# mmaker/c-lwe-snarks

Hardware: AMD Instinct MI355X
Metric: snark_proofs_per_sec (higher is better)
Workload: dtype u32 limbs (704-bit integers mod 2^704) + AES-256 bytes; int8 digits on the matrix cores, int32 accumulation (exact)

## Files before the change

### c-lwe-snarks_amd/csrc/evalmm.hip

```cpp
#include <algorithm>
#include <cstring>

#include "ctx.hpp"

namespace {

using mf::AesKey;

constexpr int CT = 4;
constexpr int SB = 88;
constexpr int VB = 92;
constexpr int MB = CT * SB;
constexpr int MT = MB / 32;
constexpr int RT = 128;
constexpr int TSTRIDE = 384;
constexpr int BLK_PER_ROW = 24;
static_assert(MB % 32 == 0 && CT * VB + 15 <= TSTRIDE, "tile geometry");

typedef int v4i __attribute__((ext_vector_type(4)));
typedef int v16i __attribute__((ext_vector_type(16)));

__device__ __forceinline__ uint32_t coef_at(const MmIo &io, uint32_t v, uint32_t nrows, uint32_t i) {
  if (io.bits) {
    const uint32_t a = io.bits_row0 + i;
// ... 244 lines not shown
    for (int q = 0; q < NT; q++)
#pragma unroll
      for (int e = 0; e < 16; e++) {
        const uint32_t mm = wave * 32 + (e & 3) + 8 * (e >> 2) + 4 * h;
        p[(uint64_t)mm * N + 32 * q + r32] = acc[q][e];
      }
  }
}

constexpr int RT2 = 256, TS2 = 192, BPR2 = 12, NQ2 = 16, N2 = 16 * NQ2;
template <int LOGQ> struct W16;
template <> struct W16<736> { static constexpr int CT = 2, SBY = 88, VBY = 92, MT = 11, MBP = 176, LL = 12; };
template <> struct W16<1472> { static constexpr int CT = 1, SBY = 184, VBY = 184, MT = 12, MBP = 192, LL = 23; };
static_assert(RT2 * 4 == 1024 && BPR2 % 4 == 0 && RT2 * BPR2 == 3 * 1024 && W16<736>::CT * W16<736>::VBY + 8 <= TS2 && W16<1472>::CT * W16<1472>::VBY + 8 <= TS2, "wide tile geometry");

template <int MODE, int LOGQ>
__global__ __launch_bounds__(1024) void k_evalmm16(AesKey key , const uint32_t *__restrict__ g_t0, uint64_t off,
                                                   uint32_t n, uint32_t nrows, uint32_t rows_per_chunk, const uint8_t *__restrict__ c8,
                                                   const int8_t *__restrict__ cd, int *__restrict__ part, uint8_t *__restrict__ image) {
  using G = W16<LOGQ>;
  constexpr int CT2 = G::CT, MT2 = G::MT, MB2 = G::MBP, NSW = (16 - G::MT) * 64;
  constexpr uint32_t SBq = G::SBY, VBq = G::VBY;
  struct __attribute__((aligned(16))) Lds {
    uint32_t lt[mf::kTabBytes / 4];
    uint8_t tile[RT2 * TS2];
    v4i bfrag[2][NQ2][64];
    uint32_t spanc[RT2][2][5];
  };
  __shared__ Lds lds;
  mf::lds_fill_tab(lds.lt, g_t0);
  const uint8_t *tab = reinterpret_cast<const uint8_t *>(lds.lt);
  const mf::AesLane L = mf::aes_lane();
  const uint32_t tid = threadIdx.x, lane = tid & 63, wave = tid >> 6;
  const uint32_t j0 = blockIdx.x * CT2;
  const uint32_t nks = j0 >= n ? 0u : min((uint32_t)CT2, n - j0);
  const bool has_b = j0 + CT2 > n && j0 <= n;
  const uint32_t r0 = blockIdx.y * rows_per_chunk;
  const uint32_t r1 = min(nrows, r0 + rows_per_chunk);

  v4i acc[NQ2];
#pragma unroll
  for (int q = 0; q < NQ2; q++) acc[q] = v4i{0, 0, 0, 0};

  const uint32_t c16 = lane & 15, g4 = lane >> 4;
  const uint32_t m = wave * 16 + c16;
  const uint32_t mcol = (m / SBq) * VBq + (m % SBq);
  const uint32_t hstep = (n * VBq) & 15;

  auto span_task = [&](uint32_t u0, uint32_t task) {
    const uint32_t lr = task >> 1, which = task & 1;
    const uint64_t row = (uint64_t)u0 + lr;
    if (row >= r1 || !nks) return;
    const RowGeom g = row_geom(off, row, n, j0, nks, VBq);
    const uint64_t sp0 = g.cb0 >> 8, sp1 = (g.cb0 + g.nblk - 1) >> 8;
    if (which && sp1 == sp0) return;
    uint32_t sc[5];
    mf::aes_span_consts(tab, L, key, sp0 + which, sc);
#pragma unroll
    for (int i = 0; i < 5; i++) lds.spanc[lr][which][i] = sc[i];
  };
  const v4i *cdv = reinterpret_cast<const v4i *>(cd);
  const uint32_t KS = (nrows + RT2 - 1) / RT2 * (RT2 / 64);

  __syncthreads();
  if (tid < 2 * RT2) span_task(r0, tid);
  __syncthreads();
  for (uint32_t u0 = r0; u0 < r1; u0 += RT2) {
    if (MODE == 1) {
      for (uint32_t s2 = tid; s2 < RT2 * BPR2; s2 += 1024) {
        const uint32_t lr = s2 / BPR2, k = s2 % BPR2;
        const uint64_t row = (uint64_t)u0 + lr;
        uint32_t w[4] = {0x80808080u, 0x80808080u, 0x80808080u, 0x80808080u};
        if (row < r1) {
          const RowGeom g = row_geom(off, row, n, j0, nks, VBq);
          if (k < g.nblk) {
            const uint64_t ctr = g.cb0 + k;
            const uint32_t *scp = lds.spanc[lr][(uint32_t)((ctr >> 8) - (g.cb0 >> 8))];
            uint32_t sc[5] = {scp[0], scp[1], scp[2], scp[3], scp[4]};
            mf::aes256_ctr_block_sc(tab, L, key, ctr, sc, w);
          }
        }
        *reinterpret_cast<uint4 *>(&lds.tile[lr * TS2 + 16 * k]) = make_uint4(w[0], w[1], w[2], w[3]);
      }
      __syncthreads();
      if (has_b) {
        for (uint32_t s2 = tid; s2 < RT2 * VBq; s2 += 1024) {
          const uint32_t lr = s2 / VBq, k = s2 % VBq;
          const uint64_t row = (uint64_t)u0 + lr;
          if (row >= r1) continue;
          const RowGeom g = row_geom(off, row, n, j0, nks, VBq);
          lds.tile[lr * TS2 + g.head + nks * VBq + k] = (uint8_t)(c8[row * VBq + k] ^ 0x80);
        }
        __syncthreads();
      }
      if (wave < MT2) {
        const uint32_t head0 = row_geom(off, u0, n, j0, 1, VBq).head;
        v4i *dst = reinterpret_cast<v4i *>(image) + ((uint64_t)(MT2 * blockIdx.x + wave) * KS + (u0 >> 6)) * 64 + lane;
#pragma unroll
        for (int ks = 0; ks < RT2 / 64; ks++) {
          const uint32_t lrb = ks * 64 + 16 * g4;
          uint32_t aw[4];
#pragma unroll
          for (int e4 = 0; e4 < 4; e4++) {
            uint32_t x = 0;
#pragma unroll
            for (int e = 0; e < 4; e++) {
              const uint32_t lr = lrb + 4 * e4 + e;
              x |= (uint32_t)lds.tile[lr * TS2 + ((head0 + hstep * lr) & 15) + mcol] << (8 * e);
            }
            aw[e4] = x;
          }
          dst[(uint64_t)ks * 64] = v4i{(int)aw[0], (int)aw[1], (int)aw[2], (int)aw[3]};
        }
      } else {
        const uint32_t t2 = tid - MT2 * 64;
        for (uint32_t task = t2; task < 2 * RT2; task += NSW) span_task(u0 + RT2, task);
      }
      __syncthreads();
      continue;
    }
    const v4i bstage = cdv[(uint64_t)(u0 >> 6) * NQ2 * 64 + tid];
    if (wave >= MT2) {
      const uint32_t t2 = tid - MT2 * 64;
#pragma unroll
      for (int k2 = 1; k2 < RT2 / 64; k2++)
#pragma unroll
        for (int i2 = 0; i2 < 4; i2++) {
          const uint32_t idx = t2 + NSW * i2;
          if (idx < NQ2 * 64) acc[(k2 - 1) * 4 + i2] = cdv[((uint64_t)(u0 >> 6) + k2) * NQ2 * 64 + idx];
        }
    }
    {
      const uint32_t lr = tid >> 2;
      const uint64_t row = (uint64_t)u0 + lr;
      if (row < r1) {
        const RowGeom g = row_geom(off, row, n, j0, nks, VBq);
#pragma unroll 1
        for (int it = 0; it < BPR2 / 4; it++) {
          const uint32_t k = (tid & 3) + 4 * it;
          if (k >= g.nblk) continue;
          const uint64_t ctr = g.cb0 + k;
          const uint32_t *scp = lds.spanc[lr][(uint32_t)((ctr >> 8) - (g.cb0 >> 8))];
          uint32_t sc[5] = {scp[0], scp[1], scp[2], scp[3], scp[4]};
          uint32_t w[4];
          mf::aes256_ctr_block_sc(tab, L, key, ctr, sc, w);
          *reinterpret_cast<uint4 *>(&lds.tile[lr * TS2 + 16 * k]) = make_uint4(w[0], w[1], w[2], w[3]);
        }
      }
    }
    (&lds.bfrag[0][0][0])[tid] = bstage;
    __syncthreads();
    if (has_b) {
      for (uint32_t s2 = tid; s2 < RT2 * VBq; s2 += 1024) {
        const uint32_t lr = s2 / VBq, k = s2 % VBq;
        const uint64_t row = (uint64_t)u0 + lr;
        if (row >= r1) continue;
        const RowGeom g = row_geom(off, row, n, j0, nks, VBq);
        lds.tile[lr * TS2 + g.head + nks * VBq + k] = (uint8_t)(c8[row * VBq + k] ^ 0x80);
      }
      __syncthreads();
    }
    const uint32_t head0 = row_geom(off, u0, n, j0, 1, VBq).head;
#pragma unroll
    for (int ks = 0; ks < RT2 / 64; ks++) {
      if (wave < MT2) {
        if ((uint64_t)u0 + ks * 64 < r1) {
          const uint32_t lrb = ks * 64 + 16 * g4;
          uint32_t aw[4];
#pragma unroll
          for (int e4 = 0; e4 < 4; e4++) {
            uint32_t x = 0;
#pragma unroll
            for (int e = 0; e < 4; e++) {
              const uint32_t lr = lrb + 4 * e4 + e;
              x |= (uint32_t)lds.tile[lr * TS2 + ((head0 + hstep * lr) & 15) + mcol] << (8 * e);
            }
            aw[e4] = x;
          }
          const v4i a = {(int)aw[0], (int)aw[1], (int)aw[2], (int)aw[3]};
#ifndef MM_SKIP_MFMA
#pragma unroll
          for (int q = 0; q < NQ2; q++) acc[q] = __builtin_amdgcn_mfma_i32_16x16x64_i8(a, lds.bfrag[ks & 1][q][lane], acc[q], 0, 0, 0);
#else
          acc[0][0] += a[0] + a[1] + a[2] + a[3];
#endif
        }
      } else {
        const uint32_t t2 = tid - MT2 * 64;
        if (ks + 1 < RT2 / 64) {
          v4i *dst = &lds.bfrag[(ks + 1) & 1][0][0];
#pragma unroll
          for (int i2 = 0; i2 < 4; i2++) {
            const uint32_t idx = t2 + NSW * i2;
            if (idx < NQ2 * 64) dst[idx] = acc[ks * 4 + i2];
          }
        }
        if (ks == 0)
          for (uint32_t task = t2; task < 2 * RT2; task += NSW) span_task(u0 + RT2, task);
      }
      __syncthreads();
    }
  }
  if (MODE == 0 && wave < MT2) {
    int *p = part + ((uint64_t)blockIdx.y * gridDim.x + blockIdx.x) * MB2 * N2;
#pragma unroll
    for (int q = 0; q < NQ2; q++)
#pragma unroll
      for (int e = 0; e < 4; e++) p[(uint64_t)(wave * 16 + 4 * g4 + e) * N2 + 16 * q + c16] = acc[q][e];
  }
}


#ifndef MMS_SW
#define MMS_SW 8
#endif
constexpr int SW = MMS_SW;
constexpr int TPW = 16;
#ifndef MMS_RQ
#define MMS_RQ 2
#endif
constexpr int RQ = MMS_RQ;
constexpr int RG = 16 / RQ;
constexpr int CG = SW / RG;
constexpr int CH = NQ2 / CG;
struct MmsImages { const v4i *image[16]; };
__device__ __forceinline__ void mms_item(uint32_t xcd, uint32_t slot, uint32_t ngt, uint32_t ngr, uint32_t map, uint32_t &grp, uint32_t &tg) {
  if (map == 0) {
    grp = slot % ngt;
    tg = (slot / ngt) * 8 + xcd;
  } else {
    const uint32_t blk = slot >> 5, i = slot & 31, nreg = ngt / ngr, tpb = 32 / ngr;
    grp = (blk % nreg) * ngr + i % ngr;
    tg = ((blk / nreg) * tpb + i / ngr) * 8 + xcd;
  }
}
__device__ __forceinline__ long long mms_pack_e(const v4i &a) {
  return (long long)a[0] + ((long long)a[1] << 8) + ((long long)a[2] << 16) + ((long long)a[3] << 24);
}
template <int CTRL>
__device__ __forceinline__ long long mms_quad_bcast(long long t) {
  const int lo = __builtin_amdgcn_update_dpp(0, (int)(unsigned int)(unsigned long long)t, CTRL, 0xf, 0xf, false);
  const int hi = __builtin_amdgcn_update_dpp(0, (int)((unsigned long long)t >> 32), CTRL, 0xf, 0xf, false);
  return (long long)(((unsigned long long)(unsigned int)hi << 32) | (unsigned int)lo);
}
__device__ __forceinline__ void mms_store_packed(int *__restrict__ part, uint32_t pk, uint64_t m4 , uint32_t ctile, uint32_t c16,
                                                 const v4i &acc) {
  const long long T = mms_pack_e(acc);
  if (pk == 1) {
    reinterpret_cast<long long *>(part)[m4 * N2 + 16 * ctile + c16] = T;
    return;
  }
  const long long T1 = mms_quad_bcast<0x55>(T), T2 = mms_quad_bcast<0xAA>(T), T3 = mms_quad_bcast<0xFF>(T);
  if (c16 & 3) return;
  const __int128 U = (__int128)T + (__int128)T1 * 256 + (__int128)T2 * 65536 + (__int128)T3 * 16777216;
  const unsigned __int128 u = (unsigned __int128)U;
  reinterpret_cast<uint4 *>(part)[m4 * (N2 / 4) + 4 * ctile + (c16 >> 2)] = uint4{(uint32_t)u, (uint32_t)(u >> 32), (uint32_t)(u >> 64), 0u};
}
__device__ __forceinline__ void mmstream_body(const MmsImages &imgs, uint32_t mtiles, uint32_t KS, uint32_t nrows, uint32_t rows_per_chunk,
                                              const v4i *__restrict__ cdv, int *__restrict__ part, uint32_t grp, uint32_t tg ,
                                              uint32_t chunk, uint64_t cd_stride , uint64_t part_stride , uint32_t pk ) {
  __shared__ v4i bfrag[2][RT2 / 64][NQ2][64];
  const uint32_t tid = threadIdx.x, lane = tid & 63;
  const uint32_t wave = __builtin_amdgcn_readfirstlane(tid >> 6);
  const uint32_t c16 = lane & 15, g4 = lane >> 4;
  const uint32_t rq = wave % RG, ch = wave / RG;
  if (tg * 16 >= mtiles) return;
  const v4i *__restrict__ image = imgs.image[grp];
  cdv += grp * cd_stride;
  part += grp * part_stride;
  const uint32_t mt0 = (tg * RG + rq) * RQ;
  const uint32_t r0 = chunk * rows_per_chunk, r1 = min(nrows, r0 + rows_per_chunk);
  v4i acc[RQ][CH];
#pragma unroll
  for (int t = 0; t < RQ; t++)
#pragma unroll
    for (int q = 0; q < CH; q++) acc[t][q] = v4i{0, 0, 0, 0};
  constexpr int KSN = RT2 / 64;
  constexpr int BPK = NQ2 * 64 / (SW * 64);
#ifndef MMS_DEPTH
#define MMS_DEPTH 6
#endif
  constexpr int DEPTH = MMS_DEPTH;
  auto a_load = [&](int t, uint32_t u0, int ks) -> v4i {
#ifdef MMS_SKIP_A
    return v4i{(int)u0, ks, t, (int)lane};
#endif
    const v4i *ap = image + ((uint64_t)min(mt0 + t, mtiles - 1) * KS + (u0 >> 6) + ks) * 64;
    return ap[lane];
  };
  v4i a[RQ][KSN];
  v4i bnr[KSN][BPK];
  auto b_load = [&](uint32_t u0, int ks, int i) -> v4i {
    const v4i *bp = cdv + (uint64_t)(u0 >> 6) * NQ2 * 64 + (uint64_t)ks * NQ2 * 64 + SW * 64 * i;
    return bp[tid];
  };
  if (r0 >= r1) return;
  const uint32_t ulast = r0 + (r1 - r0 - 1) / RT2 * RT2;
#pragma unroll
  for (int i = 0; i < KSN * BPK; i++) (&bfrag[0][0][0][0])[tid + SW * 64 * i] = cdv[(uint64_t)(r0 >> 6) * NQ2 * 64 + tid + SW * 64 * i];
  __builtin_amdgcn_sched_barrier(0);
#pragma unroll
  for (int ks = 0; ks < KSN; ks++) {
#pragma unroll
    for (int t = 0; t < RQ; t++) a[t][ks] = a_load(t, r0, ks);
#pragma unroll
    for (int i = 0; i < BPK; i++) bnr[ks][i] = b_load(min(r0 + RT2, ulast), ks, i);
    __builtin_amdgcn_sched_barrier(0);
  }
  __syncthreads();
#if defined(MMS_PRIO_YOUNG)
  if (wave >= SW / 2) __builtin_amdgcn_s_setprio(1);
#elif defined(MMS_PRIO_OLD)
  if (wave < SW / 2) __builtin_amdgcn_s_setprio(1);
#endif
  uint32_t buf = 0;
  for (uint32_t u0 = r0; u0 < r1; u0 += RT2) {
    const uint32_t un1 = min(u0 + RT2, ulast), un2 = min(u0 + 2 * RT2, ulast);
    const v4i *bcur = &bfrag[buf][0][ch * CH][lane];
    v4i *bnext = &bfrag[buf ^ 1][0][0][0];
    v4i ring[DEPTH];
#pragma unroll
    for (int i = 0; i < DEPTH; i++) ring[i] = bcur[((i / CH) * NQ2 + i % CH) * 64];
#pragma unroll
    for (int ks = 0; ks < KSN; ks++) {
#ifdef MMS_LOADS_ONLY
#pragma unroll
      for (int t = 0; t < RQ; t++) acc[t][ks][0] += a[t][ks][0] ^ a[t][ks][3];
#else
#pragma unroll
      for (int q = 0; q < CH; q++) {
        const int it = ks * CH + q;
        const v4i b = ring[it % DEPTH];
        if (it + DEPTH < KSN * CH) ring[it % DEPTH] = bcur[(((it + DEPTH) / CH) * NQ2 + (it + DEPTH) % CH) * 64];
#pragma unroll
        for (int t = 0; t < RQ; t++) {
#ifdef MMS_ACC_ASM
          asm volatile("v_mfma_i32_16x16x64_i8 %0, %1, %2, %0" : "+a"(acc[t][q]) : "v"(a[t][ks]), "v"(b));
#else
          acc[t][q] = __builtin_amdgcn_mfma_i32_16x16x64_i8(a[t][ks], b, acc[t][q], 0, 0, 0);
#endif
        }
        __builtin_amdgcn_sched_barrier(0);
      }
#endif
#pragma unroll
      for (int i = 0; i < BPK; i++) bnext[ks * NQ2 * 64 + tid + SW * 64 * i] = bnr[ks][i];
#pragma unroll
      for (int t = 0; t < RQ; t++) a[t][ks] = a_load(t, un1, ks);
#pragma unroll
      for (int i = 0; i < BPK; i++) bnr[ks][i] = b_load(un2, ks, i);
    }
#ifndef MMS_NOSYNC
    __syncthreads();
#endif
    buf ^= 1;
  }
  const uint64_t Mtot = (uint64_t)mtiles * 16;
#ifdef MMS_ACC_ASM
  asm volatile("s_nop 15\n\ts_nop 15" ::: "memory");
#endif
  if (pk) {
#pragma unroll
    for (int t = 0; t < RQ; t++) {
      if (mt0 + t >= mtiles) continue;
      const uint64_t m4 = (uint64_t)chunk * (Mtot / 4) + (uint64_t)(mt0 + t) * 4 + g4;
#pragma unroll
      for (int q = 0; q < CH; q++) mms_store_packed(part, pk, m4, ch * CH + q, c16, acc[t][q]);
    }
    return;
  }
#pragma unroll
  for (int t = 0; t < RQ; t++) {
    if (mt0 + t >= mtiles) continue;
    int *p = part + ((uint64_t)chunk * Mtot + (uint64_t)(mt0 + t) * 16) * N2;
#pragma unroll
    for (int q = 0; q < CH; q++)
#pragma unroll
      for (int e = 0; e < 4; e++) p[(uint64_t)(4 * g4 + e) * N2 + 16 * (ch * CH + q) + c16] = acc[t][q][e];
  }
}

__global__ __launch_bounds__(SW * 64) void k_mmstream(MmsImages imgs, uint32_t mtiles, uint32_t KS, uint32_t nrows, uint32_t rows_per_chunk,
                                                      const v4i *__restrict__ cdv, int *__restrict__ part, uint32_t ngt, uint32_t ngr, uint32_t map,
                                                      uint64_t cd_stride, uint64_t part_stride, uint32_t pk) {
  uint32_t grp, tg;
  mms_item(blockIdx.x & 7, blockIdx.x >> 3, ngt, ngr, map, grp, tg);
  mmstream_body(imgs, mtiles, KS, nrows, rows_per_chunk, cdv, part, grp, tg, blockIdx.y, cd_stride, part_stride, pk);
}
__global__ __launch_bounds__(SW * 64) void k_mmstream1(MmsImages imgs, uint32_t mtiles, uint32_t KS, uint32_t nrows, uint32_t rows_per_chunk,
                                                       const v4i *__restrict__ cdv, int *__restrict__ part, uint32_t pk) {
  mmstream_body(imgs, mtiles, KS, nrows, rows_per_chunk, cdv, part, 0u, blockIdx.x, blockIdx.y, 0, 0, pk);
}
__device__ __forceinline__ void mmstream_persistent(const MmsImages &imgs, uint32_t mtiles, uint32_t KS, uint32_t nrows, uint32_t rows_per_chunk,
                                                    const v4i *__restrict__ cdv, int *__restrict__ part, uint32_t ngt, uint32_t ngr, uint32_t map,
                                                    uint64_t cd_stride, uint64_t part_stride, uint32_t nblk , uint32_t nchunks,
                                                    uint32_t *__restrict__ sync, uint32_t sync_mode, uint32_t spin_max, uint32_t width, uint32_t pk) {
  const uint32_t xcd = blockIdx.x & 7, cu = blockIdx.x >> 3;
  const uint32_t members = sync_mode == 2 ? 32u : (map ? ngr : ngt);
  uint32_t *ctr = sync + xcd * 32 + (sync_mode == 2 ? 0u : cu / members);
  uint32_t k = 0;
  for (uint32_t chunk = 0; chunk < nchunks; chunk++)
    for (uint32_t slot = cu; slot < nblk * 32; slot += width, k++) {
      if (sync_mode && members > 1) {
        if (threadIdx.x == 0) {
          __hip_atomic_fetch_add(ctr, 1u, __ATOMIC_RELAXED, __HIP_MEMORY_SCOPE_AGENT);
          const uint32_t target = (k + 1) * members;
          for (uint32_t spin = 0; spin < spin_max && __hip_atomic_load(ctr, __ATOMIC_RELAXED, __HIP_MEMORY_SCOPE_AGENT) < target; spin++) __builtin_amdgcn_s_sleep(8);
        }
        __syncthreads();
      }
      uint32_t grp, tg;
      mms_item(xcd, slot, ngt, ngr, map, grp, tg);
      mmstream_body(imgs, mtiles, KS, nrows, rows_per_chunk, cdv, part, grp, tg, chunk, cd_stride, part_stride, pk);
    }
}
__global__ __launch_bounds__(SW * 64) void k_mmstream_p(MmsImages imgs, uint32_t mtiles, uint32_t KS, uint32_t nrows, uint32_t rows_per_chunk,
                                                        const v4i *__restrict__ cdv, int *__restrict__ part, uint32_t ngt, uint32_t ngr, uint32_t map,
                                                        uint64_t cd_stride, uint64_t part_stride, uint32_t nblk, uint32_t nchunks,
                                                        uint32_t *__restrict__ sync, uint32_t sync_mode, uint32_t spin_max, uint32_t width, uint32_t pk) {
  mmstream_persistent(imgs, mtiles, KS, nrows, rows_per_chunk, cdv, part, ngt, ngr, map, cd_stride, part_stride, nblk, nchunks, sync, sync_mode, spin_max, width, pk);
}
__global__ __launch_bounds__(SW * 64) void k_mmstream_pb(MmsImages imgs, uint32_t mtiles, uint32_t KS, uint32_t nrows, uint32_t rows_per_chunk,
                                                         const v4i *__restrict__ cdv, int *__restrict__ part, uint32_t ngt, uint32_t ngr, uint32_t map,
                                                         uint64_t cd_stride, uint64_t part_stride, uint32_t nblk, uint32_t nchunks,
                                                         uint32_t *__restrict__ sync, uint32_t sync_mode, uint32_t spin_max, uint32_t width, uint32_t pk) {
  mmstream_persistent(imgs, mtiles, KS, nrows, rows_per_chunk, cdv, part, ngt, ngr, map, cd_stride, part_stride, nblk, nchunks, sync, sync_mode, spin_max, width, pk);
}

constexpr int WSW = 4, WRQ = 4;
__device__ __forceinline__ void mfma_acc(v4i &acc, const v4i &a, const v4i &b) {
  asm volatile("v_mfma_i32_16x16x64_i8 %0, %1, %2, %0" : "+a"(acc) : "v"(a), "v"(b));
}
__device__ __forceinline__ void mmstream_body_w(const MmsImages &imgs, uint32_t mtiles, uint32_t KS, uint32_t nrows, uint32_t rows_per_chunk,
                                                const v4i *__restrict__ cdv, int *__restrict__ part, uint32_t grp, uint32_t tg, uint32_t chunk, uint64_t cd_stride,
                                                uint64_t part_stride) {
  __shared__ v4i bfrag[2][RT2 / 64][NQ2][64];
  const uint32_t tid = threadIdx.x, lane = tid & 63;
  const uint32_t wave = __builtin_amdgcn_readfirstlane(tid >> 6);
  const uint32_t c16 = lane & 15, g4 = lane >> 4;
  if (tg * 16 >= mtiles) return;
  const v4i *__restrict__ image = imgs.image[grp];
  cdv += grp * cd_stride;
  part += grp * part_stride;
  const uint32_t mt0 = tg * 16 + wave * WRQ;
  const uint32_t r0 = chunk * rows_per_chunk, r1 = min(nrows, r0 + rows_per_chunk);
  if (r0 >= r1) return;
  constexpr int KSN = RT2 / 64;
  constexpr int BPK = NQ2 * 64 / (WSW * 64);
  v4i acc[WRQ][NQ2];
#pragma unroll
  for (int t = 0; t < WRQ; t++)
#pragma unroll
    for (int q = 0; q < NQ2; q++) acc[t][q] = v4i{0, 0, 0, 0};
  auto a_load = [&](int t, uint32_t u0, int ks) -> v4i {
    const v4i *ap = image + ((uint64_t)min(mt0 + t, mtiles - 1) * KS + (u0 >> 6) + ks) * 64;
    return ap[lane];
  };
  auto b_load = [&](uint32_t u0, int ks, int i) -> v4i {
    const v4i *bp = cdv + (uint64_t)(u0 >> 6) * NQ2 * 64 + (uint64_t)ks * NQ2 * 64 + WSW * 64 * i;
    return bp[tid];
  };
  const uint32_t ulast = r0 + (r1 - r0 - 1) / RT2 * RT2;
  v4i a[WRQ][KSN], bnr[KSN][BPK];
#pragma unroll
  for (int i = 0; i < KSN * BPK; i++) (&bfrag[0][0][0][0])[tid + WSW * 64 * i] = cdv[(uint64_t)(r0 >> 6) * NQ2 * 64 + tid + WSW * 64 * i];
  __builtin_amdgcn_sched_barrier(0);
  const uint32_t ub1 = min(r0 + RT2, ulast);
#pragma unroll
  for (int i = 0; i < BPK; i++) bnr[0][i] = b_load(ub1, 0, i);
#pragma unroll
  for (int ks = 1; ks < KSN; ks++) {
#pragma unroll
    for (int i = 0; i < BPK; i++) bnr[ks][i] = b_load(ub1, ks, i);
#pragma unroll
    for (int t = 0; t < WRQ; t++) a[t][ks - 1] = a_load(t, r0, ks - 1);
    __builtin_amdgcn_sched_barrier(0);
  }
  __syncthreads();
  v4i rg[4][4];
  uint32_t buf = 0;
  auto frag = [&](uint32_t b, int f) -> v4i { return bfrag[b][f >> 4][f & 15][lane]; };
#pragma unroll
  for (int G = 0; G < 2; G++)
#pragma unroll
    for (int j = 0; j < 4; j++) rg[G][j] = frag(0, 4 * G + j);
  for (uint32_t u0 = r0; u0 < r1; u0 += RT2) {
    const uint32_t un1 = min(u0 + RT2, ulast), un2 = min(u0 + 2 * RT2, ulast);
    v4i *bnext = &bfrag[buf ^ 1][0][0][0];
#pragma unroll
    for (int ks = 0; ks < KSN; ks++) {
#pragma unroll
      for (int g = 0; g < 4; g++) {
        const int G = ks * 4 + g, Gn = G + 2;
#pragma unroll
        for (int u = 0; u < 4; u++) {
          const int j = 3 - u;
#pragma unroll
          for (int t = WRQ - 1; t >= 0; t--) mfma_acc(acc[t][4 * g + j], a[t][ks], rg[G & 3][j]);
          rg[Gn & 3][u] = Gn < 16 ? frag(buf, 4 * Gn + u) : frag(buf ^ 1, 4 * (Gn - 16) + u);
          if (g == 0) {
            bnext[ks * NQ2 * 64 + tid + WSW * 64 * (BPK - 1 - u)] = bnr[ks][BPK - 1 - u];
          } else if (g == 1) {
            bnr[ks][u] = b_load(un2, ks, u);
          } else if (g == 2) {
            if (ks == 0) a[u][KSN - 1] = a_load(u, u0, KSN - 1);
            else a[u][ks - 1] = a_load(u, un1, ks - 1);
          }
          __builtin_amdgcn_sched_barrier(0);
        }
        if (G == 9) {
          asm volatile("s_waitcnt lgkmcnt(4)\n\ts_barrier" ::: "memory");
          __builtin_amdgcn_sched_barrier(0);
        }
      }
    }
    buf ^= 1;
  }
  __syncthreads();
  asm volatile("s_nop 15\n\ts_nop 15" ::: "memory");
  const uint64_t Mtot = (uint64_t)mtiles * 16;
#pragma unroll
  for (int t = 0; t < WRQ; t++) {
    if (mt0 + t >= mtiles) continue;
    int *p = part + ((uint64_t)chunk * Mtot + (uint64_t)(mt0 + t) * 16) * N2;
#pragma unroll
    for (int q = 0; q < NQ2; q++)
#pragma unroll
      for (int e = 0; e < 4; e++) p[(uint64_t)(4 * g4 + e) * N2 + 16 * q + c16] = acc[t][q][e];
  }
}
__global__ __launch_bounds__(WSW * 64) void k_mmstream_w(MmsImages imgs, uint32_t mtiles, uint32_t KS, uint32_t nrows, uint32_t rows_per_chunk,
                                                         const v4i *__restrict__ cdv, int *__restrict__ part, uint32_t ngt, uint32_t ngr, uint32_t map,
                                                         uint64_t cd_stride, uint64_t part_stride, uint32_t nblk, uint32_t nchunks) {
  const uint32_t xcd = blockIdx.x & 7, cu = blockIdx.x >> 3;
  for (uint32_t k = 0; k < nblk * nchunks; k++) {
    uint32_t grp, tg;
    mms_item(xcd, (k % nblk) * 32 + cu, ngt, ngr, map, grp, tg);
    mmstream_body_w(imgs, mtiles, KS, nrows, rows_per_chunk, cdv, part, grp, tg, k / nblk, cd_stride, part_stride);
  }
}

template <int ND, int KWM ,
          bool PK >
__device__ __forceinline__ void evalmm_finish_body(const int *__restrict__ part, const int64_t *__restrict__ sc, uint32_t nchunks, uint32_t ntiles, uint32_t N,
                                                   uint32_t nvec, uint32_t n, uint32_t nrows, uint32_t ct, uint32_t MBv, uint32_t sby, uint32_t LL,
                                                   const MmIo &io, int accumulate, const int *__restrict__ sa_part, uint32_t sa_col) {
  __shared__ uint32_t sv[KWM][3][64];
  const uint32_t vl = threadIdx.x & 63, lq = threadIdx.x >> 6;
  const uint32_t v = blockIdx.y * 64 + vl, j = blockIdx.x;
  const uint32_t tile = j / ct, jj = j % ct;
  const uint32_t KWv = sby / 4;
  if (v < nvec) {
    int64_t corr[ND];
#pragma unroll
    for (int w = 0; w < ND; w++) corr[w] = 128 * sc[ND * v + w] + 16384ll * nrows;
    if (PK) {
      const uint64_t M4 = (uint64_t)ntiles * MBv / 4;
      unsigned __int128 corrsum = 0;
#pragma unroll
      for (int w = 0; w < ND; w++) corrsum += (unsigned __int128)((uint64_t)corr[w] * 0x01010101ull) << (8 * w);
      for (uint32_t l = lq; l < KWv; l += 4) {
        const uint64_t m4 = ((uint64_t)tile * MBv + jj * sby) / 4 + l;
        __int128 U = 0, SA = 0;
        for (uint32_t ch = 0; ch < nchunks; ch++) {
          const uint64_t at = (uint64_t)ch * M4 + m4;
          if (ND == 4) {
            const uint4 r = reinterpret_cast<const uint4 *>(part)[at * (N / 4) + v], q = reinterpret_cast<const uint4 *>(sa_part)[at * (N / 4) + sa_col / 4];
            U += (__int128)(((unsigned __int128)(uint64_t)(int64_t)(int32_t)r.z << 64) | ((uint64_t)r.y << 32) | r.x);
            SA += (__int128)(((unsigned __int128)(uint64_t)(int64_t)(int32_t)q.z << 64) | ((uint64_t)q.y << 32) | q.x);
          } else {
            U += reinterpret_cast<const long long *>(part)[at * N + v];
            SA += reinterpret_cast<const long long *>(sa_part)[at * N + sa_col];
          }
        }
        const unsigned __int128 val = (unsigned __int128)(U + SA * (__int128)(ND == 4 ? 128ll * 0x01010101ll : 128ll)) + corrsum;
        sv[l][0][vl] = (uint32_t)val;
        sv[l][1][vl] = (uint32_t)(val >> 32);
        sv[l][2][vl] = (uint32_t)(val >> 64);
      }
    } else
    for (uint32_t l = lq; l < KWv; l += 4) {
      unsigned __int128 val = 0;
      int g0[4][ND], sa0[4];
#pragma unroll
      for (int k = 0; k < 4; k++) {
        const int *row = part + ((uint64_t)tile * MBv + (jj * sby + 4 * l + k)) * N;
#pragma unroll
        for (int w = 0; w < ND; w++) g0[k][w] = row[ND * v + w];
        sa0[k] = (sa_part + ((uint64_t)tile * MBv + (jj * sby + 4 * l + k)) * N)[sa_col];
      }
#pragma unroll
      for (int k = 0; k < 4; k++) {
        const uint32_t mm = jj * sby + 4 * l + k;
        int64_t g[ND], sa = sa0[k];
#pragma unroll
        for (int w = 0; w < ND; w++) g[w] = g0[k][w];
        for (uint32_t ch = 1; ch < nchunks; ch++) {
          const int *row = part + (((uint64_t)ch * ntiles + tile) * MBv + mm) * N;
#pragma unroll
          for (int w = 0; w < ND; w++) g[w] += row[ND * v + w];
          sa += (sa_part + (((uint64_t)ch * ntiles + tile) * MBv + mm) * N)[sa_col];
        }
        uint64_t t = 0;
#pragma unroll
        for (int w = 0; w < ND; w++) t += (uint64_t)(g[w] + 128 * sa + corr[w]) << (8 * w);
        val += (unsigned __int128)t << (8 * k);
      }
      sv[l][0][vl] = (uint32_t)val;
      sv[l][1][vl] = (uint32_t)(val >> 32);
      sv[l][2][vl] = (uint32_t)(val >> 64);
    }
  }
  __syncthreads();
  if (lq != 0 || v >= nvec) return;
  uint32_t *out = reinterpret_cast<uint32_t *>((v < io.osplit ? io.out[0] + (uint64_t)v * io.ostride : io.out[1] + (uint64_t)(v - io.osplit) * io.ostride) +
                                               (uint64_t)j * LL);
  const bool wide4 = (LL & 1) == 0 && (io.ostride & 1) == 0 && ((reinterpret_cast<uintptr_t>(io.out[0]) | reinterpret_cast<uintptr_t>(io.out[1])) & 15) == 0;
  uint32_t pend[4] = {0, 0, 0, 0};
  uint64_t carry = 0;
  const uint32_t *actw = io.add_ct ? reinterpret_cast<const uint32_t *>(io.add_ct + (uint64_t)j * LL) : nullptr;
  const uint64_t ax = io.add_ct ? io.add_scale[v] : 0;
  uint64_t acarry = 0;
  for (uint32_t l = 0; l < KWv; l++) {
    uint64_t word = carry + sv[l][0][vl];
    if (l >= 1) word += sv[l - 1][1][vl];
    if (l >= 2) word += sv[l - 2][2][vl];
    if (accumulate) word += out[l];
    if (actw) {
      const uint64_t t = (uint64_t)actw[l] * ax + acarry;
      word += (uint32_t)t;
      acarry = t >> 32;
    }
    carry = word >> 32;
    pend[l & 3] = (uint32_t)word;
    if (wide4 ? (l & 3) == 3 : (l & 1) == 1) {
      if (wide4) *reinterpret_cast<uint4 *>(out + (l & ~3u)) = uint4{pend[0], pend[1], pend[2], pend[3]};
      else *reinterpret_cast<uint2 *>(out + (l & ~1u)) = uint2{pend[(l & 2)], pend[(l & 2) + 1]};
    }
  }
  if (wide4) {
    if (KWv & 3) *reinterpret_cast<uint4 *>(out + (KWv & ~3u)) = uint4{pend[0], (KWv & 3) > 1 ? pend[1] : 0u, (KWv & 3) > 2 ? pend[2] : 0u, 0u};
    for (uint32_t l = (KWv + 3) & ~3u; l < 2 * LL; l += 4) *reinterpret_cast<uint4 *>(out + l) = uint4{0u, 0u, 0u, 0u};
  } else {
    if (KWv & 1) *reinterpret_cast<uint2 *>(out + (KWv & ~1u)) = uint2{pend[(KWv & 2)], 0u};
    for (uint32_t l = (KWv + 1) & ~1u; l < 2 * LL; l += 2) *reinterpret_cast<uint2 *>(out + l) = uint2{0u, 0u};
  }
}

template <int ND, int KWM, bool PK>
__global__ __launch_bounds__(256) void k_evalmm_finish(const int *__restrict__ part, const int64_t *__restrict__ sc, uint32_t nchunks, uint32_t ntiles,
                                                        uint32_t N, uint32_t nvec, uint32_t n, uint32_t nrows, uint32_t ct, uint32_t MBv, uint32_t sby,
                                                        uint32_t LL, MmIo io, int accumulate) {
  evalmm_finish_body<ND, KWM, PK>(part, sc, nchunks, ntiles, N, nvec, n, nrows, ct, MBv, sby, LL, io, accumulate, part, ND * nvec);
}
template <int ND, int KWM, bool PK>
__global__ __launch_bounds__(256) void k_evalmm_finish_groups(const int *__restrict__ part, uint64_t part_stride, uint32_t nchunks, uint32_t ntiles, uint32_t N,
                                                               uint32_t n, uint32_t nrows, uint32_t ct, uint32_t MBv, uint32_t sby, uint32_t LL, MmGroupArgs A,
                                                               int accumulate) {
  const uint32_t g = blockIdx.z, lender = A.io[g].sa_from1 ? A.io[g].sa_from1 - 1 : g;
// ... 385 lines not shown
```

Baseline: 14000.

## Carry LDS ring prefetch across tiles and replace block sync with mid-step barrier

Hoists the B-fragment LDS ring out of the tile loop so the prefetch of the next tile's fragments overlaps the tail of the current tile. The LDS stores and global B loads are spread across the q iterations of the MFMA loop instead of being bunched after it. The end-of-tile __syncthreads is replaced by an explicit s_waitcnt lgkmcnt plus s_barrier placed at a computed slot. This is meant to hide LDS and global latency and shorten barrier stalls, but the hand-placed barrier and counter depend on static geometry assumptions and risk races if those assumptions are wrong.

```diff
diff --git a/c-lwe-snarks_amd/csrc/evalmm.hip b/c-lwe-snarks_amd/csrc/evalmm.hip
--- a/c-lwe-snarks_amd/csrc/evalmm.hip
+++ b/c-lwe-snarks_amd/csrc/evalmm.hip
@@ -570,9 +570,9 @@
 #pragma unroll
   for (int ks = 0; ks < KSN; ks++) {
 #pragma unroll
+    for (int i = 0; i < BPK; i++) bnr[ks][i] = b_load(min(r0 + RT2, ulast), ks, i);
+#pragma unroll
     for (int t = 0; t < RQ; t++) a[t][ks] = a_load(t, r0, ks);
-#pragma unroll
-    for (int i = 0; i < BPK; i++) bnr[ks][i] = b_load(min(r0 + RT2, ulast), ks, i);
     __builtin_amdgcn_sched_barrier(0);
   }
   __syncthreads();
@@ -581,25 +581,35 @@
 #elif defined(MMS_PRIO_OLD)
   if (wave < SW / 2) __builtin_amdgcn_s_setprio(1);
 #endif
+  [[maybe_unused]] constexpr int NF = KSN * CH;
+  [[maybe_unused]] constexpr int BSLOT = 2 * CH + CH - 1 - DEPTH;
+  static_assert(DEPTH >= 1 && DEPTH + BPK <= CH && 2 * BPK <= CH, "the stage barrier follows the ds_writes of its k-step and that k-step's last ring read");
+  static_assert(CH - DEPTH - BPK <= 15, "lgkmcnt is a 4-bit count");
+  v4i ring[DEPTH];
+#pragma unroll
+  for (int i = 0; i < DEPTH; i++) {
+    ring[i] = bfrag[0][i / CH][ch * CH + i % CH][lane];
+    __builtin_amdgcn_sched_barrier(0);
+  }
   uint32_t buf = 0;
   for (uint32_t u0 = r0; u0 < r1; u0 += RT2) {
     const uint32_t un1 = min(u0 + RT2, ulast), un2 = min(u0 + 2 * RT2, ulast);
-    const v4i *bcur = &bfrag[buf][0][ch * CH][lane];
+    [[maybe_unused]] const v4i *bcur = &bfrag[buf][0][ch * CH][lane];
+    [[maybe_unused]] const v4i *bnxt = &bfrag[buf ^ 1][0][ch * CH][lane];
     v4i *bnext = &bfrag[buf ^ 1][0][0][0];
-    v4i ring[DEPTH];
-#pragma unroll
-    for (int i = 0; i < DEPTH; i++) ring[i] = bcur[((i / CH) * NQ2 + i % CH) * 64];
 #pragma unroll
     for (int ks = 0; ks < KSN; ks++) {
+#pragma unroll
+      for (int q = 0; q < CH; q++) {
 #ifdef MMS_LOADS_ONLY
-#pragma unroll
-      for (int t = 0; t < RQ; t++) acc[t][ks][0] += a[t][ks][0] ^ a[t][ks][3];
+        if (q == 0) {
+#pragma unroll
+          for (int t = 0; t < RQ; t++) acc[t][ks][0] += a[t][ks][0] ^ a[t][ks][3];
+        }
 #else
-#pragma unroll
-      for (int q = 0; q < CH; q++) {
-        const int it = ks * CH + q;
+        const int it = ks * CH + q, nx = it + DEPTH;
         const v4i b = ring[it % DEPTH];
-        if (it + DEPTH < KSN * CH) ring[it % DEPTH] = bcur[(((it + DEPTH) / CH) * NQ2 + (it + DEPTH) % CH) * 64];
+        ring[it % DEPTH] = nx < NF ? bcur[((nx / CH) * NQ2 + nx % CH) * 64] : bnxt[(((nx - NF) / CH) * NQ2 + (nx - NF) % CH) * 64];
 #pragma unroll
         for (int t = 0; t < RQ; t++) {
 #ifdef MMS_ACC_ASM
@@ -608,21 +618,31 @@
           acc[t][q] = __builtin_amdgcn_mfma_i32_16x16x64_i8(a[t][ks], b, acc[t][q], 0, 0, 0);
 #endif
         }
+#endif
+        if (q < BPK) bnext[ks * NQ2 * 64 + tid + SW * 64 * q] = bnr[ks][q];
+        else if (q < 2 * BPK) bnr[ks][q - BPK] = b_load(un2, ks, q - BPK);
+#ifndef MMS_NOSYNC
+        if (ks * CH + q == BSLOT) {
+          asm volatile("s_waitcnt lgkmcnt(%0)\n\ts_barrier" ::"n"(CH - DEPTH - BPK) : "memory");
+        }
+#endif
         __builtin_amdgcn_sched_barrier(0);
       }
-#endif
-#pragma unroll
-      for (int i = 0; i < BPK; i++) bnext[ks * NQ2 * 64 + tid + SW * 64 * i] = bnr[ks][i];
 #pragma unroll
       for (int t = 0; t < RQ; t++) a[t][ks] = a_load(t, un1, ks);
-#pragma unroll
-      for (int i = 0; i < BPK; i++) bnr[ks][i] = b_load(un2, ks, i);
-    }
-#ifndef MMS_NOSYNC
-    __syncthreads();
+    }
+#ifndef MMS_LOADS_ONLY
+    if (NF % DEPTH) {
+      v4i turned[DEPTH];
+#pragma unroll
+      for (int j = 0; j < DEPTH; j++) turned[j] = ring[(NF + j) % DEPTH];
+#pragma unroll
+      for (int j = 0; j < DEPTH; j++) ring[j] = turned[j];
+    }
 #endif
     buf ^= 1;
   }
+  __syncthreads();
   const uint64_t Mtot = (uint64_t)mtiles * 16;
 #ifdef MMS_ACC_ASM
   asm volatile("s_nop 15\n\ts_nop 15" ::: "memory");
```

After: 14210, median of 6. 1.02x the previous value.
